# pangenome/allwave

Measured on AMD Instinct MI355X. Metric: aligned base-pairs/sec (whole node) + PAF lines/sec, all-pairs 10 kbp, higher is better.
Workload: dtype int16

## Files before the change

### allwave_amd/build.py

```python
import hashlib
import json
import os
import shutil
import subprocess
import tempfile
import time

ROOT = os.path.dirname(os.path.dirname(os.path.abspath(__file__)))
PKG = os.path.join(ROOT, "allwave_amd")
CSRC = os.path.join(PKG, "csrc")
HOST_DIR = os.path.join(CSRC, "host")
HIP_LIB = os.path.join(PKG, "liballwave_hip.so")
HOST_LIB = os.path.join(PKG, "liballwave_host.so")
CLI_BIN = os.path.join(PKG, "allwave_hip")
INFO = os.path.join(PKG, "BUILD_INFO.json")
ABI_HEADER = os.path.join(ROOT, "include", "allwave_hip.h")


def hipcc():
    for c in (os.environ.get("HIPCC"), shutil.which("hipcc"), "/opt/rocm/bin/hipcc"):
        if c and os.path.exists(c):
            return c
    raise RuntimeError("hipcc not found")


HIP_FLAGS = ["-O3", "-std=c++17", "--offload-arch=gfx950"]
HIP_FLAGS_AWV = HIP_FLAGS + ["-mllvm", "-amdgpu-sched-strategy=max-ilp"]
HIP_UNITS = (("engine.hip", HIP_FLAGS), ("kernels_awv.hip", HIP_FLAGS_AWV), ("planner.hip", HIP_FLAGS), ("orient.hip", HIP_FLAGS),
             ("verify.hip", HIP_FLAGS), ("clip.hip", HIP_FLAGS), ("split.hip", HIP_FLAGS), ("normalize.hip", HIP_FLAGS), ("encode.hip", HIP_FLAGS),
             ("cs.hip", HIP_FLAGS), ("coverage.hip", HIP_FLAGS), ("variants.hip", HIP_FLAGS), ("variants_fold.hip", HIP_FLAGS))
HIP_SOURCES = [os.path.join(CSRC, f) for f in ("engine.hip", "kernels_awv.hip", "kernels_awv.hpp", "biwfa_device.hpp", "range_span.hpp", "batch_plan.hpp", "twin_plan.hpp", "twin_base.hpp", "row_reuse.hpp", "planner.hip",
                                               "planner_device.hpp", "orient.hip", "orient_device.hpp", "verify.hip", "verify_device.hpp", "clip.hip", "clip_device.hpp", "clip_scan.hpp", "split.hip", "split_device.hpp", "normalize.hip", "normalize_device.hpp", "encode.hip", "encode_device.hpp", "cs.hip", "cs_device.hpp", "coverage.hip", "coverage_device.hpp", "variants.hip", "variants_fold.hip", "variants_device.hpp", "batch_items.hpp", "seq_load.hpp", "wave_ops.hpp",
                                               "host_errors.hpp", "record_pass.hpp", "record_pieces.hpp", "text_pass.hpp")] + [ABI_HEADER]


def _host_sources():
    return [os.path.join(HOST_DIR, f) for f in sorted(os.listdir(HOST_DIR)) if f.endswith((".cpp", ".hpp", ".h"))]


_VERSIONS = {}


def _tool_version(tool):
    if tool not in _VERSIONS:
        try:
            _VERSIONS[tool] = subprocess.run([tool, "--version"], stdout=subprocess.PIPE, stderr=subprocess.STDOUT).stdout.decode(errors="replace")
        except OSError:
            _VERSIONS[tool] = "?"
    return _VERSIONS[tool]


def content_hash(sources, commands, tool):
    h = hashlib.sha256()
    for s in sorted(sources):
        h.update(os.path.relpath(s, ROOT).encode() + b"\0")
        with open(s, "rb") as f:
            h.update(f.read())
        h.update(b"\0")
    for c in commands:
        h.update(" ".join(c).encode() + b"\n")
    h.update(_tool_version(tool).encode())
    return h.hexdigest()


# ... 113 lines not shown
```

### allwave_amd/csrc/biwfa_device.hpp

```cpp


#include <hip/hip_runtime.h>
#include <stdint.h>
#include <limits.h>

#include "range_span.hpp"
#include "twin_base.hpp"
#include "row_reuse.hpp"

#ifndef AWV_NS
#define AWV_NS awv
#endif
#ifndef AWV_WG
#define AWV_WG 64
#endif
namespace AWV_NS {

constexpr int WG = AWV_WG;
constexpr int MAX_SCOPE = 126;
constexpr int MAX_RING = 256;
constexpr int NCOMP = 5;
constexpr int32_t OFF_NULL = INT32_MIN / 2;
constexpr int32_t NULLISH = INT32_MIN / 4;
constexpr int32_t NULL16 = -16384;
#ifdef AWV_WIDE16
constexpr bool WENC = true;
#else
constexpr bool WENC = false;
#endif
enum { C_M = 0, C_I1 = 1, C_I2 = 2, C_D1 = 3, C_D2 = 4 };
constexpr int FALLBACK_MIN_SCORE = 250;
constexpr int FALLBACK_MIN_LENGTH = 100;
constexpr int STACK_CAP = 48;
constexpr int EV_STACK_WORDS = (STACK_CAP * 32 + 3) / 4 + 16;
constexpr int EV_TWIN_WORDS = MAX_SCOPE * NCOMP;
constexpr int SUB16_MAX_LEN = 32760;
#ifndef AWV_WAVES_PER_SIMD
#define AWV_WAVES_PER_SIMD 4
#endif
constexpr int WAVES_PER_SIMD = AWV_WAVES_PER_SIMD;
// ... 122 lines not shown
}
__device__ __forceinline__ void meta_store_scalar(RowMeta* p, int lo, int hi) {
  int l, h;
  asm("s_cmp_gt_i32 %2, %3\n\ts_cselect_b32 %0, %4, %2\n\ts_cselect_b32 %1, %5, %3" : "=&s"(l), "=&s"(h) : "s"(lo), "s"(hi), "s"(K_BIG), "s"(-K_BIG) : "scc");
  *p = RowMeta{l, h};
}
__device__ __forceinline__ void meta_store(RowMeta* p, const RowMeta& m) { *p = m; }

template <typename OffT>
struct Lds {
  typename MetaTraits<OffT>::Stored* ring_meta;
  int* bi_A;
  int* bi_oob;
  int* firstk;
  uint32_t* seq;
  RowMeta* meta_log;
};
struct PassCtx {
  unsigned long long ring_mem;
  unsigned long long ring_bytes;
  unsigned long long P[2], T[2];
  int ring, wcap;
  int x, o1, e1, o2, e2;
  int lds_meta_bytes;
  int chain_max;
  int plen, tlen, kmin[2], wcols;
  int seq_mode, p_w0, t_w0, p_bit, t_bit;
  unsigned long long meta_log;
  int wb_cap, sb_cap, end_comp;
  unsigned long long Pw, Tw;
  int multi_T, lds_seq_bytes, pb_abs, tb_abs;
  int deep_passes;
  int max_penalty, score_cap;
};
struct PhaseResult {
  int why, sc, fmax, rmax, npass;
  int sf, sr, last_fwd;
  int deep_from;
  unsigned long long cells, deep_cells;
};
struct Shared {
  Acc acc[3][2];
  int chain_maxak[2][8];
  PassCtx pctx;
  PhaseResult pres;
  Breakpoint bp_out;
  unsigned long long ext_multi;
  unsigned int win_single, win_multi, win_base, win_base_multi;
  int ext0[2];
#ifdef AWV_PROF
  unsigned long long prof[5];
#endif
  long long cur_pair;
  int error;
  int nev;
  int bt_total;
};

typedef const __attribute__((address_space(1))) uint8_t* gseq_t;
typedef uint64_t u64_unaligned __attribute__((aligned(1)));
typedef const __attribute__((address_space(1))) uint32_t* gwords_t;
__device__ __forceinline__ gseq_t to_global(const uint8_t* p) { return (gseq_t)(uintptr_t)p; }

struct SubCtx {
  int plen, tlen;
  gseq_t P[2];
// ... 2801 lines not shown
  const unsigned long long tb2 = PROF_NOW();
  if (uni(sh.error)) return uni(sh.error);
  const int nev = uni(sh.nev);
  Emit er = em;
  if (mirror) er = em_b;
  for (int e = nev - 1; e >= 0; --e) {
    const uint32_t ev = (uint32_t)uni((int)events[e]);
    const uint32_t opi = ev & 3u;
    emit_run(er, opi == 0 ? 'M' : opi == 1 ? 'X' : opi == 2 ? 'I' : 'D', (int)(ev >> 2));
  }
  if (mirror) em_b = er;
  else em = er;
  __syncthreads();
  PROF_ADD(STAT_T_EMIT, tb2);
  }
  return ST_OK;
}

constexpr int BP_OK = 0, BP_END_REACHED = 100, BP_RESTART = 101, BP_ABOVE_BOUND = 102;

template <bool P2, typename OffT>
__device__ __forceinline__ void bialign_overlap(const KParams& kp, Shared& sh, const Lds<OffT>& lds, const SubCtx& cx, void* ring_mem, rsrc_t ring_rs, int d0, int s0,
                                int s1, bool fwd, Breakpoint& bp, unsigned long long* lstats) {
  constexpr int VEC = OffTraits<OffT>::VEC;
  const DevPenalties& pn = kp.pen;
  const int d1 = 1 - d0;
  const int tid = cold_tid(), lane = tid & 63, wave = tid >> 6;
  const int rmask = kp.ring - 1;
  const int plen = cx.plen, tlen = cx.tlen, L = plen + tlen, D = tlen - plen;
  const int slot0 = s0 & rmask;
  const int A0 = uni(lds.bi_A[(d0) * kp.ring + (slot0)]), oob0 = uni(lds.bi_oob[(d0) * kp.ring + (slot0)]);
  const int kmin0 = cx.kmin[d0], kmin1 = cx.kmin[d1];
  const int Cm = D - kmin0 - kmin1;
  const int gmax = P2 ? max(pn.o1, pn.o2) : pn.o1;
  auto group_mask = [&](int ib) -> uint64_t {
    const int i = ib + lane, si = s1 - i;
    bool ok = false;
    if (i < pn.scope && si >= 0) {
      const int slot1 = si & rmask;
      ok = oob0 || lds.bi_oob[d1 * kp.ring + slot1] || (A0 + lds.bi_A[d1 * kp.ring + slot1] >= L);
    }
    return __ballot(ok);
  };
  bool any = false;
  for (int ib = 0; ib < pn.scope && !any; ib += 64) {
    uint64_t gm = group_mask(ib);
    while (gm) {
      const int i = ib + (int)__builtin_ctzll(gm);
      gm &= gm - 1;
      if (s0 + (s1 - i) - gmax < bp.score) { any = true; break; }
    }
  }
  if (!any) return;
  const bool twin = TWIN_BUILD && sizeof(OffT) == 2 && uni(sh.bp_out.comp) == TWIN_MAGIC;
  int* const lastk = twin ? (int*)(uintptr_t)(((unsigned long long)(unsigned)uni(sh.bp_out.off_r) << 32) | (unsigned)uni(sh.bp_out.off_f)) : nullptr;
  const int score_in = bp.score;
  for (int i = tid; i < pn.scope * NCOMP; i += WG) {
    lds.firstk[i] = INT_MAX;
    if (twin) __hip_atomic_store(&lastk[i], INT_MIN, __ATOMIC_RELAXED, __HIP_MEMORY_SCOPE_AGENT);
  }
  static_assert(!TWIN_BUILD || WG == 64, "the last-hit table's ordering is argued for one wave per workgroup only");
  if (twin) asm volatile("s_waitcnt vmcnt(0)" ::: "memory");
  __syncthreads();
  constexpr int ESZ = (int)sizeof(OffT);
  auto scan_all = [&](int i, int si, unsigned want) {
    int ca[NCOMP], cbn[NCOMP], so0[NCOMP], so1[NCOMP];
    unsigned live = 0;
    int chlo = INT_MAX, chhi = -1;
#pragma unroll
    for (int c = 0; c < NCOMP; ++c) {
      ca[c] = 1; cbn[c] = 0; so0[c] = so1[c] = 0;
      if (!P2 && (c == C_I2 || c == C_D2)) continue;
      if (!((want >> c) & 1u)) continue;
      const RowMeta r0 = uni(meta_load(&lds.ring_meta[(d0 * NCOMP + c) * kp.ring + slot0]));
      const RowMeta r1 = uni(meta_load(&lds.ring_meta[(d1 * NCOMP + c) * kp.ring + (si & rmask)]));
      if (row_empty(r0) || row_empty(r1)) continue;
      const int a = max(r0.lo, D - r1.hi), b = min(r0.hi, D - r1.lo);
      if (a > b) continue;
      ca[c] = a - kmin0;
      cbn[c] = b - kmin0;
      so0[c] = row_off<false, OffT>(kp, d0, c, s0);
      so1[c] = row_off<false, OffT>(kp, d1, c, si);
      live |= 1u << c;
      chlo = min(chlo, ca[c] >> 8);
      chhi = max(chhi, cbn[c] >> 8);
// ... 86 lines not shown
          }
          return cond;
        };
        int first = VEC;
#pragma unroll
        for (int j = VEC - 1; j >= 0; --j)
          if (hit(j)) first = j;
        const uint64_t mask = __ballot(first < VEC);
        if (mask) {
          const int src = (int)__builtin_ctzll(mask);
          const int fj = __builtin_amdgcn_readlane(first, src);
          if (lane == 0) atomicMin(&lds.firstk[i * NCOMP + c], cbase + src * VEC + fj + kmin0);
          if (!twin) {
            live &= ~(1u << c);
          } else {
            int last = -1;
#pragma unroll
            for (int j = 0; j < VEC; ++j)
              if (hit(j)) last = j;
            const int hsrc = 63 - (int)__builtin_clzll(mask);
            const int lj = __builtin_amdgcn_readlane(last, hsrc);
            if (lane == 0) __hip_atomic_fetch_max(&lastk[i * NCOMP + c], cbase + hsrc * VEC + lj + kmin0, __ATOMIC_RELAXED, __HIP_MEMORY_SCOPE_AGENT);
          }
        }
      }
    }
  };
  for (int ib = 0; ib < pn.scope; ib += 64) {
    uint64_t gm = group_mask(ib);
    while (gm) {
      const int i = ib + (int)__builtin_ctzll(gm);
      gm &= gm - 1;
      const int si = s1 - i;
      const bool w2 = P2 && s0 + si - pn.o2 < bp.score, w1 = s0 + si - pn.o1 < bp.score, w0 = s0 + si < bp.score;
      if (!(w2 || w1 || w0)) continue;
      scan_all(i, si, (w2 ? (1u << C_D2) | (1u << C_I2) : 0u) | (w1 ? (1u << C_D1) | (1u << C_I1) : 0u) | (w0 ? 1u << C_M : 0u));
    }
  }
  if (twin) asm volatile("s_waitcnt vmcnt(0)" ::: "memory");
  __syncthreads();
  auto apply = [&](int c, int i, int si, int gap_open) {
    const int k0 = uni(lds.firstk[i * NCOMP + c]);
    if (k0 == INT_MAX) return;
    if (s0 + si - gap_open >= bp.score) return;
    const int k1 = D - k0;
    const int32_t h0 = uni(off_load1<OffT>(row_ptr<false, OffT>(kp, ring_mem, d0, c, s0) + (k0 - kmin0), k0));
    const int32_t h1 = uni(off_load1<OffT>(row_ptr<false, OffT>(kp, ring_mem, d1, c, si) + (k1 - kmin1), k1));
    if (fwd) { bp.sf = s0; bp.sr = si; bp.kf = k0; bp.kr = k1; bp.off_f = h0; bp.off_r = h1; }
    else { bp.sf = si; bp.sr = s0; bp.kf = k1; bp.kr = k0; bp.off_f = h1; bp.off_r = h0; }
    bp.score = s0 + si - gap_open;
    bp.comp = c;
  };
  for (int ib = 0; ib < pn.scope; ib += 64) {
    uint64_t gm = group_mask(ib);
    while (gm) {
      const int i = ib + (int)__builtin_ctzll(gm);
      gm &= gm - 1;
      const int si = s1 - i;
      if (P2 && s0 + si - pn.o2 < bp.score) { apply(C_D2, i, si, pn.o2); apply(C_I2, i, si, pn.o2); }
      if (s0 + si - pn.o1 < bp.score) { apply(C_D1, i, si, pn.o1); apply(C_I1, i, si, pn.o1); }
      if (s0 + si >= bp.score) continue;
      apply(C_M, i, si, 0);
    }
  }
  if (twin) {
    Breakpoint* const rec = reinterpret_cast<Breakpoint*>(reinterpret_cast<unsigned char*>(lds.seq) - sizeof(Breakpoint));
    int tscore = uni(rec->score) == INT_MIN ? INT_MIN : score_in;
    int blk = -1, blk_v = INT_MIN;
    uint64_t blk_hits = 0;
    auto last_hit = [&](int idx) -> int {
      if ((idx >> 6) != blk) {
        blk = idx >> 6;
        const int j = (blk << 6) + lane;
        blk_v = j < pn.scope * NCOMP ? __hip_atomic_load(&lastk[j], __ATOMIC_RELAXED, __HIP_MEMORY_SCOPE_AGENT) : INT_MIN;
        blk_hits = __ballot(blk_v != INT_MIN);
      }
      if (!((blk_hits >> (idx & 63)) & 1ull)) return INT_MIN;
      return __builtin_amdgcn_readlane(blk_v, idx & 63);
    };
    auto tapply = [&](int c, int i, int si, int gap_open) {
      if (s0 + si - gap_open >= tscore) return;
      const int k0 = last_hit(i * NCOMP + c);
      if (k0 == INT_MIN) return;
      {
        const RowMeta r0 = uni(meta_load(&lds.ring_meta[(d0 * NCOMP + c) * kp.ring + slot0]));
        const RowMeta r1 = uni(meta_load(&lds.ring_meta[(d1 * NCOMP + c) * kp.ring + (si & rmask)]));
        if (k0 < r0.lo || k0 > r0.hi || D - k0 < r1.lo || D - k0 > r1.hi) {
          tscore = INT_MIN;
          if (tid == 0) rec->score = INT_MIN;
          return;
        }
      }
      const int k1 = D - k0;
      const int32_t h0 = uni(off_load1<OffT>(row_ptr<false, OffT>(kp, ring_mem, d0, c, s0) + (k0 - kmin0), k0));
      const int32_t h1 = uni(off_load1<OffT>(row_ptr<false, OffT>(kp, ring_mem, d1, c, si) + (k1 - kmin1), k1));
      tscore = s0 + si - gap_open;
      if (tid == 0) {
        const int kf = fwd ? k0 : k1, kr = fwd ? k1 : k0, hf = fwd ? h0 : h1, hr = fwd ? h1 : h0;
        rec->score = tscore;
        rec->sf = fwd ? s0 : si;
        rec->sr = fwd ? si : s0;
        rec->kf = -kf;
        rec->kr = -kr;
        rec->off_f = hf - kf;
        rec->off_r = hr - kr;
        rec->comp = twin_comp(c);
      }
    };
    for (int ib = 0; ib < pn.scope; ib += 64) {
      uint64_t gm = group_mask(ib);
      while (gm) {
        const int i = ib + (int)__builtin_ctzll(gm);
        gm &= gm - 1;
        const int si = s1 - i;
        if (P2 && s0 + si - pn.o2 < tscore) { tapply(C_I2, i, si, pn.o2); tapply(C_D2, i, si, pn.o2); }
        if (s0 + si - pn.o1 < tscore) { tapply(C_I1, i, si, pn.o1); tapply(C_D1, i, si, pn.o1); }
        if (s0 + si >= tscore) continue;
        tapply(C_M, i, si, 0);
      }
    }
  }
  __syncthreads();
}

template <bool P2, typename OffT>
__device__ __forceinline__ int find_breakpoint(const KParams& kp, Shared& sh, const Lds<OffT>& lds, SubCtx cx, void* ring_mem, rsrc_t ring_rs, int cb, int ce,
                               int score_remaining, int known_score, int attempt, Breakpoint& bp, unsigned long long* lstats) {
  const DevPenalties& pn = kp.pen;
  const int tid = cold_tid();
  const int plen = cx.plen, tlen = cx.tlen;
  const int rmask = kp.ring - 1;
  {
    long long bound = (long long)score_remaining + 2LL * pn.scope + 16;
    const long long half = (kp.wcap - 2 * COL_PAD - 9 - 256) / 2;
    bound = min(bound, half);
    const int blo = (int)min((long long)plen, bound), bhi = (int)min((long long)tlen, bound);
    const int need = -blo - 4 - COL_PAD;
    cx.kmin[0] = need;
    const int D = tlen - plen;
    const int c0 = D - need - need;
    const int adj = ((255 - c0) % 256 + 256) % 256;
    cx.kmin[1] = need - adj;
    cx.wcols = blo + bhi + 9 + adj + 2 * COL_PAD;
    if (cx.wcols > kp.wcap) return ST_CAPACITY;
  }
  const unsigned sh_addr = (unsigned)(uintptr_t)&sh, dyn_addr = (unsigned)(uintptr_t)lds.ring_meta;
  if (tid == 0) {
// ... 697 lines not shown
      cx.T[0] = to_global(Tf + t.tb);
      cx.P[1] = to_global(Pr + (plenT - t.pe));
      cx.T[1] = to_global(Tr + (tlenT - t.te));
      cx.kmin[0] = cx.kmin[1] = 0;
      cx.wcols = 0;
      cx.Pw = Pw;
      cx.Tw = Tw;
      cx.pb_abs = t.pb;
      cx.tb_abs = t.tb;
      stage_sequences<OffT>(kp, lds, cx);
      do_base = t.score_remaining <= FALLBACK_MIN_SCORE;
      if (!do_base) {
        int rc = BP_OK;
        for (int attempt = 0; attempt < AWV_RESTART_ATTEMPTS; ++attempt) {
          if (tid == 0) {
            PassCtx& pc = sh.pctx;
            pc.ring_mem = (unsigned long long)(uintptr_t)ring_mem;
            pc.ring_bytes = (unsigned long long)kp.ring_slot_stride;
            pc.P[0] = (unsigned long long)(uintptr_t)cx.P[0];
            pc.P[1] = (unsigned long long)(uintptr_t)cx.P[1];
            pc.T[0] = (unsigned long long)(uintptr_t)cx.T[0];
            pc.T[1] = (unsigned long long)(uintptr_t)cx.T[1];
            pc.Pw = (unsigned long long)(uintptr_t)cx.Pw;
            pc.Tw = (unsigned long long)(uintptr_t)cx.Tw;
            pc.ring = kp.ring;
            pc.wcap = kp.wcap;
            pc.x = pn.x; pc.o1 = pn.o1; pc.e1 = pn.e1; pc.o2 = pn.o2; pc.e2 = pn.e2;
            pc.lds_meta_bytes = kp.lds_meta_bytes;
            pc.lds_seq_bytes = kp.lds_seq_bytes;
            pc.chain_max = kp.chain_max;
            pc.multi_T = kp.multi_T;
            pc.deep_passes = kp.deep_passes;
            pc.max_penalty = kp.pair_max_penalty ? kp.pair_max_penalty[pair] : kp.max_penalty;
            pc.plen = plen; pc.tlen = tlen;
            pc.seq_mode = cx.seq_mode; pc.p_w0 = cx.p_w0; pc.t_w0 = cx.t_w0; pc.p_bit = cx.p_bit; pc.t_bit = cx.t_bit;
            pc.pb_abs = cx.pb_abs; pc.tb_abs = cx.tb_abs;
            const unsigned long long tab = (unsigned long long)(uintptr_t)(events + kp.wcap + EV_STACK_WORDS);
            sh.bp_out.comp = mode == TM_SHARED && !kp.score_only ? TWIN_MAGIC : 0;
            sh.bp_out.off_f = (int)(unsigned)tab;
            sh.bp_out.off_r = (int)(unsigned)(tab >> 32);
            if (mode == TM_SHARED)
              reinterpret_cast<Breakpoint*>(dyn_smem + kp.lds_meta_bytes - sizeof(Breakpoint))->score = INT_MAX;
          }
          __syncthreads();
          if constexpr (sizeof(OffT) == 4 && !WENC) {
            if (kp.sub16 != 0 && max(plen, tlen) < SUB16_MAX_LEN)
              rc = uni(find_breakpoint_fn<P2, int16_t>((unsigned)(uintptr_t)&sh, (unsigned)(uintptr_t)lds.ring_meta, (unsigned)(uintptr_t)lstats,
                                                       t.cb, t.ce, t.score_remaining, t.known, attempt | 0x100));
            else
              rc = uni(find_breakpoint_fn<P2, OffT>((unsigned)(uintptr_t)&sh, (unsigned)(uintptr_t)lds.ring_meta, (unsigned)(uintptr_t)lstats,
                                                    t.cb, t.ce, t.score_remaining, t.known, attempt));
          } else if (rr_hdr != nullptr) {
            int part = 0;
            if (t.score_remaining == INT_MAX) part = RR_RECORD;
            else if (rr_bv >= 0 && (mode == rr_mode || (rr_mode == TM_SHARED && mode == TM_A))) {
              if (t.pb == 0 && t.tb == 0 && t.pe == rr_bv && t.te == rr_bh && t.cb == C_M && t.ce == rr_comp) part = RR_FWD;
              else if (t.pb == rr_bv && t.tb == rr_bh && t.pe == plenT && t.te == tlenT && t.cb == rr_comp && t.ce == C_M) part = RR_REV;
            }
            if (tid == 0) {
              const unsigned long long ra = (unsigned long long)(uintptr_t)rr_hdr;
              lds.firstk[RRS_ARCH_LO] = (int)(unsigned)ra;
              lds.firstk[RRS_ARCH_HI] = (int)(unsigned)(ra >> 32);
              lds.firstk[RRS_PASSES] = rr_passes;
              lds.firstk[RRS_T] = rr_T;
              lds.firstk[RRS_NID] = rr_nid;
              lds.firstk[RRS_PART] = part;
// ... 1 lines not shown
            }
            __syncthreads();
            rc = uni(find_breakpoint_fn_reuse<P2, OffT>((unsigned)(uintptr_t)&sh, (unsigned)(uintptr_t)lds.ring_meta, (unsigned)(uintptr_t)lstats,
                                                        t.cb, t.ce, t.score_remaining, t.known, attempt));
          } else {
            rc = uni(find_breakpoint_fn<P2, OffT>((unsigned)(uintptr_t)&sh, (unsigned)(uintptr_t)lds.ring_meta, (unsigned)(uintptr_t)lstats,
                                                  t.cb, t.ce, t.score_remaining, t.known, attempt));
          }
          if (rc == BP_OK) {
            bp.score = uni(sh.bp_out.score); bp.sf = uni(sh.bp_out.sf); bp.sr = uni(sh.bp_out.sr); bp.kf = uni(sh.bp_out.kf);
            bp.kr = uni(sh.bp_out.kr); bp.off_f = uni(sh.bp_out.off_f); bp.off_r = uni(sh.bp_out.off_r); bp.comp = uni(sh.bp_out.comp);
            if (mode == TM_SHARED && !kp.score_only) {
              const Breakpoint* rec = reinterpret_cast<const Breakpoint*>(dyn_smem + kp.lds_meta_bytes - sizeof(Breakpoint));
              bq.score = uni(rec->score); bq.sf = uni(rec->sf); bq.sr = uni(rec->sr); bq.kf = uni(rec->kf);
              bq.off_f = uni(rec->off_f); bq.comp = uni(rec->comp);
            }
          }
          if (rc != BP_RESTART) break;
          if (tid == 0) lstats[STAT_RESTARTS] += 1;
        }
        if (TWINS && pair_b >= 0 && run_mode == TM_SHARED) {
          if (mode == TM_SHARED) ++tw_shared;
          else ++tw_solo;
        }
        if (rc == BP_END_REACHED) {
          if (mode == TM_SHARED) split = true;
          else do_base = true;
        }
        else if (rc == BP_ABOVE_BOUND) { status = ST_ABOVE_BOUND; break; }
        else if (rc != BP_OK) { status = rc; break; }
      }
      }
      bool shared_base = false;
      if (split && kp.twin_base != 0) {
        if (tlen == 0 || plen == 0) {
          const int n = max(plen, tlen);
          const int pen_gap = n > 0 ? min(pn.o1 + n * pn.e1, P2 ? pn.o2 + n * pn.e2 : INT_MAX) : 0;
          emit_run(em, tlen == 0 ? 'D' : 'I', n);
          emit_run(em_o, plen == 0 ? 'D' : 'I', n);
          if (top) penalty = pen_gap;
          if (top_o) penalty_o = pen_gap;
          top = top_o = false;
          continue;
        }
        if (t.score_remaining <= FALLBACK_MIN_SCORE) {
          cx.plen = plen;
          cx.tlen = tlen;
          cx.P[0] = to_global(Pf + t.pb);
          cx.T[0] = to_global(Tf + t.tb);
          cx.P[1] = to_global(Pr + (plenT - t.pe));
          cx.T[1] = to_global(Tr + (tlenT - t.te));
          cx.kmin[0] = cx.kmin[1] = 0;
          cx.wcols = 0;
          cx.Pw = Pw;
          cx.Tw = Tw;
          cx.pb_abs = t.pb;
          cx.tb_abs = t.tb;
          stage_sequences<OffT>(kp, lds, cx);
        }
        split = false;
        do_base = shared_base = true;
      }
      if (split) {
        if (sp + 2 > STACK_CAP) { status = ST_TWIN_REDO; break; }
        if (tid == 0) {
          stack[sp] = Task{t.tb, t.te, t.pb, t.pe, twin_comp(t.cb) | (TM_B << 8), twin_comp(t.ce), t.score_remaining, t.known};
          stack[sp + 1] = Task{t.pb, t.pe, t.tb, t.te, t.cb | (TM_A << 8), t.ce, t.score_remaining, t.known};
// ... 194 lines not shown
      cx.P[1] = to_global(Pr + (plenT - t.pe));
      cx.T[1] = to_global(Tr + (tlenT - t.te));
      cx.kmin[0] = cx.kmin[1] = 0;
      cx.wcols = 0;
      cx.Pw = Pw;
      cx.Tw = Tw;
      cx.pb_abs = t.pb;
      cx.tb_abs = t.tb;
      stage_sequences<OffT>(kp, lds, cx);
      bool do_base = t.score_remaining <= FALLBACK_MIN_SCORE;
      Breakpoint bp;
      if (!do_base) {
        int rc = BP_OK;
        for (int attempt = 0; attempt < AWV_RESTART_ATTEMPTS; ++attempt) {
          if (tid == 0) {
            PassCtx& pc = sh.pctx;
            pc.ring_mem = (unsigned long long)(uintptr_t)ring_mem;
            pc.ring_bytes = (unsigned long long)kp.ring_slot_stride;
            pc.P[0] = (unsigned long long)(uintptr_t)cx.P[0];
            pc.P[1] = (unsigned long long)(uintptr_t)cx.P[1];
            pc.T[0] = (unsigned long long)(uintptr_t)cx.T[0];
            pc.T[1] = (unsigned long long)(uintptr_t)cx.T[1];
            pc.Pw = (unsigned long long)(uintptr_t)cx.Pw;
            pc.Tw = (unsigned long long)(uintptr_t)cx.Tw;
            pc.ring = kp.ring;
            pc.wcap = kp.wcap;
            pc.x = pn.x; pc.o1 = pn.o1; pc.e1 = pn.e1; pc.o2 = pn.o2; pc.e2 = pn.e2;
            pc.lds_meta_bytes = kp.lds_meta_bytes;
            pc.lds_seq_bytes = kp.lds_seq_bytes;
            pc.chain_max = kp.chain_max;
            pc.multi_T = kp.multi_T;
            pc.deep_passes = kp.deep_passes;
            pc.max_penalty = kp.pair_max_penalty ? kp.pair_max_penalty[pair] : kp.max_penalty;
            pc.plen = plen; pc.tlen = tlen;
            pc.seq_mode = cx.seq_mode; pc.p_w0 = cx.p_w0; pc.t_w0 = cx.t_w0; pc.p_bit = cx.p_bit; pc.t_bit = cx.t_bit;
            pc.pb_abs = cx.pb_abs; pc.tb_abs = cx.tb_abs;
          }
          __syncthreads();
          if constexpr (sizeof(OffT) == 4 && !WENC) {
            if (kp.sub16 != 0 && max(plen, tlen) < SUB16_MAX_LEN)
              rc = uni(find_breakpoint_fn<P2, int16_t>((unsigned)(uintptr_t)&sh, (unsigned)(uintptr_t)lds.ring_meta, (unsigned)(uintptr_t)lstats,
                                                       t.cb, t.ce, t.score_remaining, t.known, attempt | 0x100));
            else
              rc = uni(find_breakpoint_fn<P2, OffT>((unsigned)(uintptr_t)&sh, (unsigned)(uintptr_t)lds.ring_meta, (unsigned)(uintptr_t)lstats,
                                                    t.cb, t.ce, t.score_remaining, t.known, attempt));
          } else {
            rc = uni(find_breakpoint_fn<P2, OffT>((unsigned)(uintptr_t)&sh, (unsigned)(uintptr_t)lds.ring_meta, (unsigned)(uintptr_t)lstats,
                                                  t.cb, t.ce, t.score_remaining, t.known, attempt));
          }
          if (rc == BP_OK) {
            bp.score = uni(sh.bp_out.score); bp.sf = uni(sh.bp_out.sf); bp.sr = uni(sh.bp_out.sr); bp.kf = uni(sh.bp_out.kf);
            bp.kr = uni(sh.bp_out.kr); bp.off_f = uni(sh.bp_out.off_f); bp.off_r = uni(sh.bp_out.off_r); bp.comp = uni(sh.bp_out.comp);
          }
          if (rc != BP_RESTART) break;
          if (tid == 0) lstats[STAT_RESTARTS] += 1;
        }
        if (rc == BP_END_REACHED) do_base = true;
        else if (rc == BP_ABOVE_BOUND) { status = ST_ABOVE_BOUND; break; }
        else if (rc != BP_OK) { status = rc; break; }
      }
      if (do_base) {
        int pen_b = 0;
        const int rc = base_align<P2, OffT>(kp, sh, lds, cx, hist, hist_rs, events, t.cb, t.ce, em, pen_b, lstats);
        if (rc != ST_OK) { status = rc; break; }
        if (top) penalty = pen_b;
        top = false;
// ... 63 lines not shown
```

### allwave_amd/csrc/engine.hip

```cpp
#include "allwave_hip.h"
#include "host_errors.hpp"
#include "planner_device.hpp"
#include "verify_device.hpp"
#include "clip_device.hpp"
#include "split_device.hpp"
#include "normalize_device.hpp"
#include "encode_device.hpp"
#include "cs_device.hpp"
#include "coverage_device.hpp"
#include "variants_device.hpp"
#include "kernels_awv.hpp"
#define AWV_NS awv
#define AWV_WG 64
#include "biwfa_device.hpp"
#undef AWV_NS
#undef AWV_WG
#define AWV_NS awvw
#define AWV_WG 256
#include "biwfa_device.hpp"
#undef AWV_NS
#undef AWV_WG
#define AWV_NS awvx
#define AWV_WG 1024
#include "biwfa_device.hpp"
// ... 557 lines not shown
  nunits = (int64_t)m;
  if (rp.twin_here)
    if (int rc = upload_twin_units(c, ge, nunits)) return rc;
  AWV_TRY(hipMemsetAsync(e->d_counters.p, 0, (1 + awv::STAT_N_DEV + awv::RR_DESC_WORDS) * sizeof(unsigned long long), e->stream));
  if (c.reuse.passes > 0) {
    st.hreuse[0] = (unsigned long long)(uintptr_t)e->reuse_mem.p;
    st.hreuse[1] = (unsigned long long)c.reuse.bytes();
    st.hreuse[2] = (unsigned long long)(unsigned)c.reuse.passes | ((unsigned long long)(unsigned)c.reuse.T << 32);
    st.hreuse[3] = (unsigned long long)c.reuse.nid;
    AWV_TRY(hipMemcpyAsync(e->d_counters.p + 1 + awv::STAT_N_DEV, st.hreuse, sizeof(st.hreuse), hipMemcpyHostToDevice, e->stream));
  }
  return timer_stop(c, c.h2d_ms);
}

awv::KParams fill_kparams(const AlignCall& c, const awvb::RowPlan& rp, int wc, int64_t nunits) {
  const awv_engine* e = c.e;
  const SeqSet& s = c.s;
  const bool narrow = rp.width != 1;
  awv::KParams kp{};
  for (int v = 0; v < 4; ++v) kp.seq[v] = s.d_seq[v].p;
  kp.seq_off = s.d_off.p;
  kp.seq_len = s.d_len.p;
  kp.seq2[0] = s.d_seq2[0].p;
  kp.seq2[1] = s.d_seq2[1].p;
  kp.seq2_off = s.d_off2.p;
  kp.seq2_ok = s.d_ok2.p;
  kp.pair_q = e->d_pair_q.p;
  kp.pair_t = e->d_pair_t.p;
  kp.pair_rc = e->d_pair_rc.p;
  kp.npairs = nunits;
  kp.unit_first = rp.twin_here ? e->d_unit_first.p : nullptr;
  kp.unit_twin = rp.twin_here ? e->d_unit_twin.p : nullptr;
  kp.twin_levels = (e->cfg.flags & AWV_F_TWIN_TOP_ONLY) ? 1 : INT_MAX;
  kp.twin_base = (e->cfg.flags & AWV_F_NO_TWIN_BASE) ? 0 : 1;
  kp.pen = awv::DevPenalties{c.pp.x, c.pp.o1, c.pp.e1, c.pp.o2, c.pp.e2, c.pp.two_piece, c.pp.scope};
  kp.ring = c.pp.ring;
  kp.multi_T = narrow ? c.pp.multi_T : (std::min(c.pp.multi_T, awv::TMAX32) >= 2 ? std::min(c.pp.multi_T, awv::TMAX32) : 0);
  kp.deep_passes = (kp.multi_T > 0 && !(e->cfg.flags & AWV_F_NO_DEEP)) ? 1 : 0;
  kp.sub16 = (e->cfg.flags & AWV_F_FORCE_INT32) ? 0 : 1;
  kp.chain_max = narrow ? c.pp.chain_max : (awv::TMAX32 == awv::TMAX ? std::min(c.pp.chain_max, 3) : 1);
  kp.wcap = wc;
  kp.ring_mem = e->ring_mem.p;
  kp.ring_slot_stride = rp.ring_stride(wc);
  kp.lds_meta_bytes = (int)rp.lds_meta;
  kp.lds_seq_bytes = (int)rp.lds_seq;
  kp.sb_cap = c.pp.sb_cap;
  kp.wb_cap = c.pp.wb_cap;
  kp.hist_mem = e->hist_mem.p;
  kp.hist_slot_stride = rp.hist_stride;
  kp.hist_meta_offset = rp.hist_rows;
  kp.ev_mem = e->ev_mem.p;
  kp.ev_slot_stride = rp.ev_stride(wc);
  kp.cigar = e->d_cigar.p;
  kp.cigar_off = e->d_cigar_off.p;
  kp.results = e->d_results.p;
  kp.work_counter = e->d_counters.p;
  kp.stats = e->d_counters.p + 1;
  kp.score_only = c.rq.score_only ? 1 : 0;
  kp.max_penalty = c.rq.max_penalty;
  kp.pair_max_penalty = c.rq.pair_bound ? e->d_pair_bound.p : nullptr;
  return kp;
}

struct LaunchShape {
  unsigned grid;
  int wg;
  size_t dyn_lds;
// ... 760 lines not shown
```

### allwave_amd/ffi.py

```python
import ctypes as C
import os

import numpy as np

_HERE = os.path.dirname(os.path.abspath(__file__))
LIB_PATH = os.environ.get("AWV_HIP_LIB") or os.path.join(_HERE, "liballwave_hip.so")

AWV_OK = 0
AWV_ERR_NO_DEVICE = -1
AWV_ERR_ARG = -3
AWV_ERR_STATE = -6
AWV_ERR_SINK = -7
AWV_ST_COMPLETED = 0
AWV_ST_CAPACITY = 1
AWV_ST_ABOVE_BOUND = 4
AWV_F_KEEP_ON_DEVICE = 1
AWV_F_FORCE_INT32 = 2
AWV_F_NO_PACKED_SEQ = 4
AWV_F_ONE_WAVE = 8
AWV_F_FOUR_WAVES = 16
AWV_F_NO_ARENA_PROBE = 32
AWV_F_SINGLE_STEP = 64
AWV_F_NO_CHAIN = 128
AWV_F_NO_WIDE16 = 256
AWV_F_NO_DEEP = 512
AWV_F_NO_RERUN = 1024
AWV_F_NO_TWIN = 2048
AWV_F_TWIN_TOP_ONLY = 4096
AWV_F_NO_TWIN_BASE = 8192
AWV_F_NO_ROW_REUSE = 16384
AWV_ORIENT_FORWARD = 0
AWV_ORIENT_REVERSE = 1
AWV_ORIENT_UNDECIDED = 2
AWV_ORIENT_BY_BOUND = 0
AWV_ORIENT_BY_EDITS = 1
AWV_ORIENT_FULL = 1
AWV_ORIENT_SKIP_RATIO = 8
AWV_ORIENT_NO_EDITS = 2 ** 64 - 1
AWV_ORIENT_HI_NONE = 2 ** 31 - 1
AWV_VF_OK = 0
AWV_VF_SKIPPED = 1
AWV_VF_BAD_OP = 2
AWV_VF_OVERRUN = 3
AWV_VF_M_DIFFERS = 4
AWV_VF_X_EQUAL = 5
AWV_VF_SHORT = 6
AWV_VF_COUNTS = 7
AWV_VF_PENALTY = 8
AWV_CL_OK = 0
AWV_CL_SKIPPED = 1
AWV_CL_EMPTY = 2
AWV_CL_BAD_OP = 3
AWV_CLIP_MAX_BONUS = 32767
AWV_NORM_OFF = 0
AWV_NORM_LEFT = 1
AWV_NORM_RIGHT = 2
AWV_NM_OK = 0
AWV_NM_SKIPPED = 1
AWV_NM_BAD_OP = 2
AWV_NM_LENGTHS = 3
AWV_CS_SHORT = 1
AWV_CS_LONG = 2
AWV_CST_OK = 0
# ... 977 lines not shown
```

### include/allwave_hip.h

```cpp
#ifndef ALLWAVE_HIP_H
#define ALLWAVE_HIP_H

#include <stddef.h>
#include <stdint.h>

#ifdef __cplusplus
extern "C" {
#endif

#define AWV_ABI_VERSION 3

#define AWV_OK 0
#define AWV_ERR_NO_DEVICE (-1)
#define AWV_ERR_HIP (-2)
#define AWV_ERR_ARG (-3)
#define AWV_ERR_PENALTIES (-4)
#define AWV_ERR_OOM (-5)
#define AWV_ERR_STATE (-6)
#define AWV_ERR_SINK (-7)

#define AWV_ST_COMPLETED 0
#define AWV_ST_CAPACITY 1
#define AWV_ST_INTERNAL 2
#define AWV_ST_MAX_STEPS 3
#define AWV_ST_ABOVE_BOUND 4

typedef struct awv_engine awv_engine;

typedef struct {
  int32_t device;
  int32_t workgroups;
  int64_t max_batch_pairs;
  int64_t max_arena_bytes;
  int32_t flags;
  int32_t first_row_cols;
  int64_t max_scratch_bytes;
} awv_engine_config;

#define AWV_F_KEEP_ON_DEVICE 1
#define AWV_F_NO_ARENA_PROBE 32
#define AWV_F_NO_RERUN 1024
#define AWV_F_FORCE_INT32 2
#define AWV_F_NO_WIDE16 256
#define AWV_F_NO_PACKED_SEQ 4
#define AWV_F_ONE_WAVE 8
#define AWV_F_FOUR_WAVES 16
#define AWV_F_NO_CHAIN 128
#define AWV_F_NO_DEEP 512
#define AWV_F_SINGLE_STEP 64
#define AWV_F_NO_TWIN 2048
#define AWV_F_TWIN_TOP_ONLY 4096
#define AWV_F_NO_TWIN_BASE 8192
#define AWV_F_NO_ROW_REUSE 16384

typedef struct {
  int32_t match;
  int32_t mismatch;
  int32_t gap_open1;
  int32_t gap_ext1;
  int32_t gap_open2;
  int32_t gap_ext2;
  int32_t two_piece;
} awv_penalties;

typedef struct {
  int32_t q_idx;
  int32_t t_idx;
  int32_t q_revcomp;
} awv_pair;

typedef struct {
  int32_t status;
  int32_t penalty;
  int32_t score;
  uint32_t cigar_len;
  uint64_t cigar_off;
  int32_t num_matches;
  int32_t num_mismatches;
  int32_t num_ins;
  int32_t num_del;
  int32_t q_end;
  int32_t t_end;
} awv_result;

typedef int (*awv_sink)(void* user, int64_t first, int64_t n, const awv_result* results,
                        const uint8_t* cigar_arena);
// ... 418 lines not shown
```

Before: 782.0 million.

## Prune BiWFA breakpoint scans using a known lower bound on the score

Passes a per-task known score lower bound into the phase context and uses it to skip breakpoint-overlap candidates whose score cannot reach that bound, both in the barrier check, the finalize scan and the twin apply path. Out-of-bounds diagonals disable the pruning for safety. A new flag AWV_F_NO_KNOWN_BOUND disables it via bit 2 of twin_base, and a scratch script compares outputs with and without. It adds extra per-candidate branching and relies on the bound being correct.

```diff
diff --git a/allwave_amd/build.py b/allwave_amd/build.py
--- a/allwave_amd/build.py
+++ b/allwave_amd/build.py
@@ -29,7 +29,7 @@
 HIP_UNITS = (("engine.hip", HIP_FLAGS), ("kernels_awv.hip", HIP_FLAGS_AWV), ("planner.hip", HIP_FLAGS), ("orient.hip", HIP_FLAGS),
              ("verify.hip", HIP_FLAGS), ("clip.hip", HIP_FLAGS), ("split.hip", HIP_FLAGS), ("normalize.hip", HIP_FLAGS), ("encode.hip", HIP_FLAGS),
              ("cs.hip", HIP_FLAGS), ("coverage.hip", HIP_FLAGS), ("variants.hip", HIP_FLAGS), ("variants_fold.hip", HIP_FLAGS))
-HIP_SOURCES = [os.path.join(CSRC, f) for f in ("engine.hip", "kernels_awv.hip", "kernels_awv.hpp", "biwfa_device.hpp", "range_span.hpp", "batch_plan.hpp", "twin_plan.hpp", "twin_base.hpp", "row_reuse.hpp", "planner.hip",
+HIP_SOURCES = [os.path.join(CSRC, f) for f in ("engine.hip", "kernels_awv.hip", "kernels_awv.hpp", "biwfa_device.hpp", "range_span.hpp", "batch_plan.hpp", "twin_plan.hpp", "twin_base.hpp", "row_reuse.hpp", "known_bound.hpp", "planner.hip",
                                                "planner_device.hpp", "orient.hip", "orient_device.hpp", "verify.hip", "verify_device.hpp", "clip.hip", "clip_device.hpp", "clip_scan.hpp", "split.hip", "split_device.hpp", "normalize.hip", "normalize_device.hpp", "encode.hip", "encode_device.hpp", "cs.hip", "cs_device.hpp", "coverage.hip", "coverage_device.hpp", "variants.hip", "variants_fold.hip", "variants_device.hpp", "batch_items.hpp", "seq_load.hpp", "wave_ops.hpp",
                                                "host_errors.hpp", "record_pass.hpp", "record_pieces.hpp", "text_pass.hpp")] + [ABI_HEADER]
 
diff --git a/allwave_amd/csrc/biwfa_device.hpp b/allwave_amd/csrc/biwfa_device.hpp
--- a/allwave_amd/csrc/biwfa_device.hpp
+++ b/allwave_amd/csrc/biwfa_device.hpp
@@ -6,6 +6,7 @@
 
 #include "range_span.hpp"
 #include "twin_base.hpp"
+#include "known_bound.hpp"
 #include "row_reuse.hpp"
 
 #ifndef AWV_NS
@@ -194,6 +195,7 @@
   int multi_T, lds_seq_bytes, pb_abs, tb_abs;
   int deep_passes;
   int max_penalty, score_cap;
+  int known_lo;
 };
 struct PhaseResult {
   int why, sc, fmax, rmax, npass;
@@ -3061,7 +3063,15 @@
   const int A0 = uni(lds.bi_A[(d0) * kp.ring + (slot0)]), oob0 = uni(lds.bi_oob[(d0) * kp.ring + (slot0)]);
   const int kmin0 = cx.kmin[d0], kmin1 = cx.kmin[d1];
   const int Cm = D - kmin0 - kmin1;
-  const int gmax = P2 ? max(pn.o1, pn.o2) : pn.o1;
+  const int klo = uni(sh.pctx.known_lo);
+  auto want_of = [&](int si) -> unsigned {
+    int lo = klo;
+    if (lo != awvkb::NONE && (oob0 || uni(lds.bi_oob[d1 * kp.ring + (si & rmask)]))) lo = awvkb::NONE;
+    const bool w2 = P2 && s0 + si - pn.o2 < bp.score && awvkb::reaches(lo, s0, si, pn.o2);
+    const bool w1 = s0 + si - pn.o1 < bp.score && awvkb::reaches(lo, s0, si, pn.o1);
+    const bool w0 = s0 + si < bp.score && awvkb::reaches(lo, s0, si, 0);
+    return (w2 ? (1u << C_D2) | (1u << C_I2) : 0u) | (w1 ? (1u << C_D1) | (1u << C_I1) : 0u) | (w0 ? 1u << C_M : 0u);
+  };
   auto group_mask = [&](int ib) -> uint64_t {
     const int i = ib + lane, si = s1 - i;
     bool ok = false;
@@ -3072,14 +3082,23 @@
     return __ballot(ok);
   };
   bool any = false;
+#ifdef AWV_DIAG
+  bool any_unbounded = false;
+#endif
   for (int ib = 0; ib < pn.scope && !any; ib += 64) {
     uint64_t gm = group_mask(ib);
     while (gm) {
       const int i = ib + (int)__builtin_ctzll(gm);
       gm &= gm - 1;
-      if (s0 + (s1 - i) - gmax < bp.score) { any = true; break; }
-    }
-  }
+#ifdef AWV_DIAG
+      if (s0 + (s1 - i) - (P2 ? max(pn.o1, pn.o2) : pn.o1) < bp.score) any_unbounded = true;
+#endif
+      if (want_of(s1 - i)) { any = true; break; }
+    }
+  }
+#ifdef AWV_DIAG
+  if (!any && any_unbounded && tid == 0) lstats[STAT_T_BI_BARRIER] += 1;
+#endif
   if (!any) return;
   const bool twin = TWIN_BUILD && sizeof(OffT) == 2 && uni(sh.bp_out.comp) == TWIN_MAGIC;
   int* const lastk = twin ? (int*)(uintptr_t)(((unsigned long long)(unsigned)uni(sh.bp_out.off_r) << 32) | (unsigned)uni(sh.bp_out.off_f)) : nullptr;
@@ -3232,9 +3251,12 @@
       const int i = ib + (int)__builtin_ctzll(gm);
       gm &= gm - 1;
       const int si = s1 - i;
-      const bool w2 = P2 && s0 + si - pn.o2 < bp.score, w1 = s0 + si - pn.o1 < bp.score, w0 = s0 + si < bp.score;
-      if (!(w2 || w1 || w0)) continue;
-      scan_all(i, si, (w2 ? (1u << C_D2) | (1u << C_I2) : 0u) | (w1 ? (1u << C_D1) | (1u << C_I1) : 0u) | (w0 ? 1u << C_M : 0u));
+      const unsigned want = want_of(si);
+      if (!want) continue;
+#ifdef AWV_DIAG
+      if (tid == 0) lstats[STAT_T_BI_FINALIZE] += 1;
+#endif
+      scan_all(i, si, want);
     }
   }
   if (twin) asm volatile("s_waitcnt vmcnt(0)" ::: "memory");
@@ -3278,8 +3300,10 @@
       if (!((blk_hits >> (idx & 63)) & 1ull)) return INT_MIN;
       return __builtin_amdgcn_readlane(blk_v, idx & 63);
     };
+    int tlo = awvkb::NONE;
     auto tapply = [&](int c, int i, int si, int gap_open) {
       if (s0 + si - gap_open >= tscore) return;
+      if (!awvkb::reaches(tlo, s0, si, gap_open)) return;
       const int k0 = last_hit(i * NCOMP + c);
       if (k0 == INT_MIN) return;
       {
@@ -3313,6 +3337,8 @@
         const int i = ib + (int)__builtin_ctzll(gm);
         gm &= gm - 1;
         const int si = s1 - i;
+        tlo = klo;
+        if (tlo != awvkb::NONE && (oob0 || uni(lds.bi_oob[d1 * kp.ring + (si & rmask)]))) tlo = awvkb::NONE;
         if (P2 && s0 + si - pn.o2 < tscore) { tapply(C_I2, i, si, pn.o2); tapply(C_D2, i, si, pn.o2); }
         if (s0 + si - pn.o1 < tscore) { tapply(C_I1, i, si, pn.o1); tapply(C_D1, i, si, pn.o1); }
         if (s0 + si >= tscore) continue;
@@ -4076,6 +4102,7 @@
             pc.multi_T = kp.multi_T;
             pc.deep_passes = kp.deep_passes;
             pc.max_penalty = kp.pair_max_penalty ? kp.pair_max_penalty[pair] : kp.max_penalty;
+            pc.known_lo = (t.known == INT_MAX || (kp.twin_base & 2)) ? awvkb::NONE : t.known;
             pc.plen = plen; pc.tlen = tlen;
             pc.seq_mode = cx.seq_mode; pc.p_w0 = cx.p_w0; pc.t_w0 = cx.t_w0; pc.p_bit = cx.p_bit; pc.t_bit = cx.t_bit;
             pc.pb_abs = cx.pb_abs; pc.tb_abs = cx.tb_abs;
@@ -4143,7 +4170,7 @@
       }
       }
       bool shared_base = false;
-      if (split && kp.twin_base != 0) {
+      if (split && (kp.twin_base & 1) != 0) {
         if (tlen == 0 || plen == 0) {
           const int n = max(plen, tlen);
           const int pen_gap = n > 0 ? min(pn.o1 + n * pn.e1, P2 ? pn.o2 + n * pn.e2 : INT_MAX) : 0;
@@ -4404,6 +4431,7 @@
             pc.multi_T = kp.multi_T;
             pc.deep_passes = kp.deep_passes;
             pc.max_penalty = kp.pair_max_penalty ? kp.pair_max_penalty[pair] : kp.max_penalty;
+            pc.known_lo = (t.known == INT_MAX || (kp.twin_base & 2)) ? awvkb::NONE : t.known;
             pc.plen = plen; pc.tlen = tlen;
             pc.seq_mode = cx.seq_mode; pc.p_w0 = cx.p_w0; pc.t_w0 = cx.t_w0; pc.p_bit = cx.p_bit; pc.t_bit = cx.t_bit;
             pc.pb_abs = cx.pb_abs; pc.tb_abs = cx.tb_abs;
diff --git a/allwave_amd/csrc/engine.hip b/allwave_amd/csrc/engine.hip
--- a/allwave_amd/csrc/engine.hip
+++ b/allwave_amd/csrc/engine.hip
@@ -613,7 +613,7 @@
   kp.unit_first = rp.twin_here ? e->d_unit_first.p : nullptr;
   kp.unit_twin = rp.twin_here ? e->d_unit_twin.p : nullptr;
   kp.twin_levels = (e->cfg.flags & AWV_F_TWIN_TOP_ONLY) ? 1 : INT_MAX;
-  kp.twin_base = (e->cfg.flags & AWV_F_NO_TWIN_BASE) ? 0 : 1;
+  kp.twin_base = ((e->cfg.flags & AWV_F_NO_TWIN_BASE) ? 0 : 1) | ((e->cfg.flags & AWV_F_NO_KNOWN_BOUND) ? 2 : 0);
   kp.pen = awv::DevPenalties{c.pp.x, c.pp.o1, c.pp.e1, c.pp.o2, c.pp.e2, c.pp.two_piece, c.pp.scope};
   kp.ring = c.pp.ring;
   kp.multi_T = narrow ? c.pp.multi_T : (std::min(c.pp.multi_T, awv::TMAX32) >= 2 ? std::min(c.pp.multi_T, awv::TMAX32) : 0);
diff --git a/allwave_amd/csrc/known_bound.hpp b/allwave_amd/csrc/known_bound.hpp
--- /dev/null
+++ b/allwave_amd/csrc/known_bound.hpp
@@ -0,0 +1,36 @@
+#pragma once
+#include <limits.h>
+
+#if defined(__HIPCC__) || defined(__CUDACC__)
+#define AWVKB_HD __host__ __device__ inline
+#else
+#define AWVKB_HD inline
+#endif
+
+namespace awvkb {
+
+constexpr int NONE = INT_MIN;
+
+AWVKB_HD bool reaches(int K, int s0, int si, int gap_open) { return s0 + si - gap_open >= K; }
+
+AWVKB_HD int last_candidate(int K, int s0, int s1, int gap_open, int scope) {
+  if (K == NONE) return scope - 1;
+  const long long i = (long long)s0 + s1 - gap_open - K;
+  return i < 0 ? -1 : i < scope - 1 ? (int)i : scope - 1;
+}
+
+AWVKB_HD bool call_empty(int K, int s0, int s1) { return last_candidate(K, s0, s1, 0, 1) < 0; }
+
+AWVKB_HD int first_id_score(int K, int scope, int open_min) {
+  if (K == NONE) return 0;
+  const long long s = ((long long)K + open_min - (scope - 1)) / 2;
+  return s < 0 ? 0 : (int)s;
+}
+
+AWVKB_HD int id_rows_after(int K, int scope, int open_min, int T) {
+  const int s = first_id_score(K, scope, open_min);
+  if (T < 1 || s < 1) return 0;
+  return (s - 1) / T * T;
+}
+
+}
diff --git a/allwave_amd/ffi.py b/allwave_amd/ffi.py
--- a/allwave_amd/ffi.py
+++ b/allwave_amd/ffi.py
@@ -29,6 +29,7 @@
 AWV_F_TWIN_TOP_ONLY = 4096
 AWV_F_NO_TWIN_BASE = 8192
 AWV_F_NO_ROW_REUSE = 16384
+AWV_F_NO_KNOWN_BOUND = 32768
 AWV_ORIENT_FORWARD = 0
 AWV_ORIENT_REVERSE = 1
 AWV_ORIENT_UNDECIDED = 2
diff --git a/include/allwave_hip.h b/include/allwave_hip.h
--- a/include/allwave_hip.h
+++ b/include/allwave_hip.h
@@ -52,6 +52,7 @@
 #define AWV_F_TWIN_TOP_ONLY 4096
 #define AWV_F_NO_TWIN_BASE 8192
 #define AWV_F_NO_ROW_REUSE 16384
+#define AWV_F_NO_KNOWN_BOUND 32768
 
 typedef struct {
   int32_t match;
diff --git a/scratch/known_bound_settings.py b/scratch/known_bound_settings.py
--- /dev/null
+++ b/scratch/known_bound_settings.py
@@ -0,0 +1,24 @@
+import json, os, sys
+sys.path.insert(0, os.path.dirname(os.path.dirname(os.path.abspath(__file__))))
+from allwave_amd import ffi, synth
+steps = int(sys.argv[1])
+cfg = synth.CONFIGS[sys.argv[2] if len(sys.argv) > 2 else "c2"]
+data, offs, _ = synth.generate(cfg["nseq"], cfg["length"], cfg["d"], cfg["seed"])
+pairs = synth.all_pairs(cfg["nseq"])
+eng = {name: ffi.Engine(flags=ffi.AWV_F_KEEP_ON_DEVICE | f) for name, f in (("default", 0), ("pinned", ffi.AWV_F_NO_KNOWN_BOUND))}
+sums = {}
+for name, e in eng.items():
+    e.set_sequences((data, offs))
+    e.align_pairs(cfg["scores"], pairs, want_cigars=False)
+for _ in range(steps):
+    for name, e in eng.items():
+        res, _ = e.align_pairs(cfg["scores"], pairs, want_cigars=False)
+        st = e.stats()
+        assert (res["status"] == 0).all()
+        sums.setdefault(name, set()).add((int(res["penalty"].sum()), int(res["cigar_len"].sum())))
+        print(json.dumps({"setting": name, "kernel_ms": st.kernel_ms, "cell_steps": int(st.cell_steps), "multi_cell_steps": int(st.multi_cell_steps),
+                          "deep_cell_steps": int(st.deep_cell_steps), "restarts": int(st.restarts), "n_breakpoints": int(st.n_breakpoints),
+                          "n_base": int(st.n_base), "overlap_scans": int(st.overlap_scans)}), flush=True)
+assert sums["default"] == sums["pinned"] and len(sums["default"]) == 1, sums
+for e in eng.values():
+    e.close()
```

Result: no change. 783.2 million (median of 5 runs) (+0.2%).
